# yuki-inaho/APDe-MVS

Measured on AMD Instinct MI355X. Metric: Mpix/s per PatchMatch iteration (ref view, N src) at 1/2/4/8 GPU; depth L1 vs ref, higher is better.
Workload: dtype f32

## Files before the change

### apde-mvs_amd/csrc/apd_kernels.hip

```cpp
#include <hip/hip_runtime.h>

#include <algorithm>
#include <cmath>
#include <cstdio>
#include <cstring>
#include <string>
#include <atomic>
#include <vector>

#include "../../include/apd_hip.h"
#include "apd_device.h"
#include <rocprim/device/device_scan.hpp>

using namespace apd;

#define WAVE 64
#define BLOCK 256
#define APD_PROF_SLOTS 64
#define APD_INSTR 32
#define APD_PROF_SPREAD 64
#define PROF_AT(ev, k) ((ev) + (k) + APD_PROF_SLOTS * (blockIdx.x & (APD_PROF_SPREAD - 1)))
#ifdef APD_PHASE_STAMPS
#define PHASE_STAMP(i)                                                                       \
    do {                                                                                     \
// ... 180 lines not shown
        const unsigned long long m = __ballot(p);
        const int pre = __popcll(m & ((1ull << lane) - 1ull));
        if (lane == 0) wcnt[wv] = __popcll(m);
        __syncthreads();
        int wo = 0;
        for (int k = 0; k < wv; ++k) wo += wcnt[k];
        const int tot = wcnt[0] + wcnt[1] + wcnt[2] + wcnt[3];
        if (mode == 2) {
            if (x < a.W) out[y * a.W + x] = p ? off + wo + pre : -1;
        } else if (p) {
            out[off + wo + pre] = y * a.W + x;
        }
        off += tot;
        __syncthreads();
    }
}

#define TILE_POS 256
#ifndef TILE_SUPER_PX
#define TILE_SUPER_PX 128
#endif
__device__ __forceinline__ void tile_coords(int t, int tiles_x, int tiles_y, int tw, int &tx, int &ty) {
    const int SX = TILE_SUPER_PX ? max(1, TILE_SUPER_PX / tw) : tiles_x;
    const int SY = TILE_SUPER_PX ? max(1, TILE_SUPER_PX / (TILE_POS / tw)) : 1;
    const int sy = t / (SY * tiles_x);
    const int rows = min(SY, tiles_y - SY * sy);
    const int r = t - sy * SY * tiles_x;
    const int sx = r / (rows * SX);
    const int cols = min(SX, tiles_x - SX * sx);
    const int r2 = r - sx * rows * SX;
    tx = SX * sx + r2 % cols;
    ty = SY * sy + r2 / cols;
}
__device__ __forceinline__ void tile_pixel(int tile, int tiles_x, int tiles_y, int tw, int k, int &x, int &y) {
    const int micro = k >> 4, inner = k & 15, mx = tw >> 2;
    const int lx = ((micro % mx) << 2) + (inner & 3);
    const int ly = ((micro / mx) << 2) + (inner >> 2);
    int tx, ty;
    tile_coords(tile, tiles_x, tiles_y, tw, tx, ty);
    x = tx * tw + lx;
    y = ty * (TILE_POS / tw) + ly;
}
__global__ __launch_bounds__(BLOCK) void k_tile_count(Args a, int mode, int colour, int tiles_x, int tw,
                                                    int *__restrict__ counts) {
    int x, y;
    tile_pixel(blockIdx.x, tiles_x, (int)gridDim.x / tiles_x, tw, threadIdx.x, x, y);
    const bool p = x < a.W && y < a.H && list_pred(a, mode, colour, x, y);
    __shared__ int wsum[BLOCK / WAVE];
    const int c = __popcll(__ballot(p));
    if ((threadIdx.x & 63) == 0) wsum[threadIdx.x >> 6] = c;
    __syncthreads();
    if (threadIdx.x == 0) counts[blockIdx.x] = wsum[0] + wsum[1] + wsum[2] + wsum[3];
}
__global__ __launch_bounds__(BLOCK) void k_tile_fill(Args a, int mode, int colour, int tiles_x, int tw,
                                                   const int *__restrict__ offs, int *__restrict__ out) {
    int x, y;
    tile_pixel(blockIdx.x, tiles_x, (int)gridDim.x / tiles_x, tw, threadIdx.x, x, y);
    const bool p = x < a.W && y < a.H && list_pred(a, mode, colour, x, y);
    __shared__ int wcnt[BLOCK / WAVE];
    const int lane = threadIdx.x & 63, wv = threadIdx.x >> 6;
    const unsigned long long m = __ballot(p);
    if (lane == 0) wcnt[wv] = __popcll(m);
    __syncthreads();
    int wo = 0;
    for (int k = 0; k < wv; ++k) wo += wcnt[k];
    const int pos = offs[blockIdx.x] + wo + __popcll(m & ((1ull << lane) - 1ull));
    if (mode == 2) {
        if (x < a.W && y < a.H) out[y * a.W + x] = p ? pos : -1;
    } else if (p) {
        out[pos] = y * a.W + x;
    }
}
__global__ __launch_bounds__(BLOCK) void k_anchor_export(Args a, const int *__restrict__ row_off, short2 *__restrict__ dst) {
    const int y = blockIdx.x;
    __shared__ int wcnt[BLOCK / WAVE];
    int off = row_off[y];
    const int lane = threadIdx.x & 63, wv = threadIdx.x >> 6;
    for (int x0 = 0; x0 < a.W; x0 += BLOCK) {
        const int x = x0 + threadIdx.x;
        const int wi = x < a.W ? a.amap[y * a.W + x] : -1;
        const unsigned long long m = __ballot(wi >= 0);
        if (lane == 0) wcnt[wv] = __popcll(m);
        __syncthreads();
        int wo = 0;
        for (int k = 0; k < wv; ++k) wo += wcnt[k];
        const int tot = wcnt[0] + wcnt[1] + wcnt[2] + wcnt[3];
        if (wi >= 0) {
            const int r = off + wo + __popcll(m & ((1ull << lane) - 1ull));
#pragma unroll
            for (int k = 0; k < 9; ++k) dst[(size_t)r * 9 + k] = a.anchors[(size_t)wi * 9 + k];
// ... 1562 lines not shown
            strong_weight += 1.0f;
        }
    }
    if (dead) return APD_COST_MAX;
    if (strong_weight <= 1e-6f) return center_cost;
    float mx = -1e10f;
#pragma unroll
    for (int t = 0; t < 9; ++t) if (t < ns && sc[t] > mx) mx = sc[t];
    float e[9];
    float sum = 0.0f;
#pragma unroll
    for (int t = 0; t < 9; ++t) {
        if (t < ns) { e[t] = d_expf(sc[t] - mx); sum += e[t]; }
    }
    float acc = 0.0f;
#pragma unroll
    for (int t = 0; t < 9; ++t) {
        if (t < ns) { float w = e[t] / sum; acc = fmaf(w, sc[t], acc); }
    }
    acc = (acc > APD_COST_MAX) ? APD_COST_MAX : acc;
    return (float)(0.25 * (double)center_cost + 0.75 * (double)acc);
}

#ifndef WV_WAVES
#define WV_WAVES 4
#endif
#ifndef WV_CUR_MATCH
#define WV_CUR_MATCH 1
#endif
#ifndef WV_P2_GEOM_BATCH
#define WV_P2_GEOM_BATCH 0
#endif
#define WV_BLOCK (WV_WAVES * WAVE)
template <bool F16, bool SA> struct WvOcc {
#ifdef WV_LDS_OCC
    static constexpr int occ = WV_LDS_OCC;
#else
    static constexpr int occ = F16 ? 4 : 3;
#endif
    static constexpr bool pipe = occ < 4 && WV_CENTRE_PIPE;
};
template <bool F16, bool SA>
__global__ __launch_bounds__(WV_BLOCK, (WvOcc<F16, SA>::occ)) void k_sweep_weak_vm(Args a, const int *__restrict__ list, int count,
                                                                int iter, const float *__restrict__ cand, int wc) {
    const int N = a.N, W = a.W;
    constexpr bool PIPE = WvOcc<F16, SA>::pipe;
    PHASE_BEGIN;
    const bool direct = cand != nullptr;
    WvLdsT<F16, 9, SA> &L = *reinterpret_cast<WvLdsT<F16, 9, SA> *>(apd_dyn_lds);
    wv_init_lut(L);
    float *costL = reinterpret_cast<float *>(&L + 1);
    uint8_t *wts = reinterpret_cast<uint8_t *>(costL + wv_cost_rows(N, direct) * VM_P);
    uint8_t *asl = wts + N * VM_P;
    const int VB = min(WV_P5_CHUNKS, N);
    const int blk = xcd_remap(blockIdx.x, gridDim.x);
    const int first = blk * VM_P;
    const int np = min(VM_P, count - first);
    const int tid = threadIdx.x;
    const int wave = __builtin_amdgcn_readfirstlane(tid >> 6), lane = tid & (WAVE - 1);
    const APD_C Cam &cam0 = a.cams[0];
    const bool geom = a.geom != 0;
    const float gf = a.gf;
    const int p1 = lane;
    const bool pv1 = p1 < np;
    const int c1 = list[first + min(p1, np - 1)];
    const int py1 = c1 / W, px1 = c1 - py1 * W;

    if (pv1) {
        const APD_G short2 *anc = a.anchors + (size_t)a.amap[c1] * 9;
        const int cid = a.sa_any ? a.sa[c1] : 0;
        const bool use_sa = cid != 0;
        if (wave == 0) {
            uint32_t hflag = 0, awin = 0;
            short2 ap[9];
#pragma unroll
            for (int k = 0; k < 9; ++k) ap[k] = anc[k];
            int lab[9], qk[9];
// ... 78 lines not shown
        const float4 pl = L.hyp[h * VM_P + p1];
        const float nv = ncc_new_vm<F16, SA, true, 9, PIPE>(a, L, p1, px1, py1, v + 1, pl, want, nullptr, &nwc, &nwa);
        if (want) val = nv;
        costL[t * VM_P + p1] = val;
    }
    __syncthreads();
    PHASE_STAMP(1);

    const int Gp = WAVE / N;
    const int ppr = WV_WAVES * Gp;
    for (int r0 = 0; r0 < np; r0 += ppr) {
        int g = lane / N;
        const bool lane_ok = g < Gp;
        int v = lane - g * N;
        if (!lane_ok) { g = 0; v = (lane - Gp * N) % N; }
        Group G;
        G.v = v; G.base = g * N; G.slot = g; G.li = 0;
        G.gmask = (N >= 64) ? ~0ull : ((1ull << N) - 1ull);
        const int pr = r0 + wave * Gp + g;
        G.valid = lane_ok && pr < np;
        const int p = min(pr, np - 1);
        const int c = list[first + p];
        const int py = c / W, px = c - py * W;
        const uint32_t hflag = L.flags[p] & 0x1FFu;
        float prior = 0.0f;
        const uint32_t asv = asl[v * VM_P + p];
#pragma unroll
        for (int i = 0; i < 8; ++i) {
            const int pk = L.anc[(i + 1) * VM_P + p];
            if (pk >= 0) prior += ((asv >> i) & 1u) ? 0.9f : 0.1f;
        }
        float ca[8];
        if (direct) {
            const size_t wi = (size_t)a.amap[c];
#pragma unroll
            for (int h = 0; h < 8; ++h)
                ca[h] = ((hflag >> h) & 1u) ? cand[((size_t)v * 8 + h) * (size_t)wc + wi] : ((h == 0 && v == 0) ? 2.0f : 0.0f);
        } else {
#pragma unroll
            for (int h = 0; h < 8; ++h) ca[h] = costL[(h * N + v) * VM_P + p];
        }
        Rng rg(a.seed_lo, a.seed_hi, (uint32_t)c, ord_weak(iter));
        const int w = view_selection(ca, prior, iter, rg, G, N);
        const uint32_t tsel = group_bits(w > 0, G);
        float gval[8];
#ifdef APD_PHASE_STAMPS
        const long long tg0_ = clock64();
#endif
#if WV_P2_GEOM_BATCH
        if (geom && w > 0) {
            GeomHead gh[8];
            float sdep[8];
#pragma unroll
            for (int j = 0; j < 8; ++j) {
                float P[3];
                geom_point(a, px, py, L.hyp[j * VM_P + p], P);
                gh[j] = geom_head(a, v + 1, P);
            }
#pragma unroll
            for (int j = 0; j < 8; ++j) sdep[j] = ((hflag >> j) & 1u) ? a.depth[gh[j].idx] : 0.0f;
#pragma unroll
            for (int j = 0; j < 8; ++j)
                gval[j] = ((hflag >> j) & 1u) ? fmaf(gf, geom_tail(a, px, py, v + 1, gh[j], sdep[j]), ca[j]) : fmaf(gf, 3.0f, ca[j]);
        } else {
#pragma unroll
            for (int j = 0; j < 8; ++j) gval[j] = ca[j];
        }
#else
        const bool share_p = geom && N >= 8;
        float Pv[3] = {0.0f, 0.0f, 0.0f};
// ... 801 lines not shown
    float4 *dst = reinterpret_cast<float4 *>(pcost + (size_t)i0 * Np);
    for (int j = threadIdx.x; j < nq; j += BLOCK) dst[j] = src[j];
}

__device__ __forceinline__ float gp_combine(float cc, const float (&sc)[8]) {
    if (cc < 0.0f) return APD_COST_MAX;
    const float center_cost = cc;
    uint32_t pm = 0;
    float strong_weight = 0.0f;
#pragma unroll
    for (int k = 0; k < 8; ++k)
        if (sc[k] >= 0.0f) { pm |= 1u << k; strong_weight += 1.0f; }
    if (strong_weight <= 1e-6f) return center_cost;
    float mx = -1e10f;
#pragma unroll
    for (int k = 0; k < 8; ++k) if (((pm >> k) & 1u) && sc[k] > mx) mx = sc[k];
    float e[8];
    float sum = 0.0f;
#pragma unroll
    for (int k = 0; k < 8; ++k) {
        e[k] = 0.0f;
        if ((pm >> k) & 1u) { e[k] = d_expf(sc[k] - mx); sum += e[k]; }
    }
    float acc = 0.0f;
#pragma unroll
    for (int k = 0; k < 8; ++k)
        if ((pm >> k) & 1u) { const float w = e[k] / sum; acc = fmaf(w, sc[k], acc); }
    acc = (acc > APD_COST_MAX) ? APD_COST_MAX : acc;
    return (float)(0.25 * (double)center_cost + 0.75 * (double)acc);
}

template <bool F16, bool SA>
__global__ __launch_bounds__(PK_BLOCK, PK_MINW) void k_weak_cand_g(Args a, const int *__restrict__ list, int count,
                                                          const uint8_t *__restrict__ cbw, float *__restrict__ out, int wc) {
    using TT = FastTex<F16, true>;
    using RT = typename std::conditional<F16, _Float16, float>::type;
    __shared__ RT cref[36 * VM_P];
    __shared__ float csr[VM_P], csrr[VM_P];
    __shared__ uint64_t cmask[VM_P];
    __shared__ uint8_t cws[VM_P], cbits[VM_P];
    __shared__ int anc0[VM_P];
    const int N = a.N, W = a.W, H = a.H;
    const int blk = xcd_remap(blockIdx.x, gridDim.x);
    const int first = blk * VM_P;
    const int np = min(VM_P, count - first);
    const int tid = threadIdx.x;
    const int wave = __builtin_amdgcn_readfirstlane(tid >> 6), lane = tid & (WAVE - 1);
    const int p1 = lane;
    const bool pv1 = p1 < np;
    const int c1 = list[first + min(p1, np - 1)];
    const int py1 = c1 / W, px1 = c1 - py1 * W;
    const int wi1 = a.amap[c1];
    const int cid = a.sa_any ? (int)a.sa[c1] : 0;
    const APD_G short2 *anc1 = a.anchors + (size_t)wi1 * 9;
    if (wave == 0) {
        int a0 = -1;
        uint32_t cb = 0;
        if (pv1) {
            const short2 z = anc1[0];
            const bool ok = !(z.x == -1 || z.y == -1) && (cid == 0 || (int)a.sa[z.x + z.y * W] == cid);
            a0 = ok ? ((int)(uint16_t)z.x | ((int)z.y << 16)) : -1;
            cb = cbw[wi1];
        }
        anc0[p1] = a0;
        cbits[p1] = (uint8_t)cb;
    }
    __syncthreads();
// ... 37 lines not shown
        const short2 ap = anc1[h + 1];
        pl = a.plane[ap.x + ap.y * W];
    }
    const int pk0 = anc0[p1];
    const uint64_t tm = SA ? cmask[p1] : ~0ull;
    uint32_t nlive = 0;
    for (int v = 0; v < N; ++v) {
        const int s = v + 1;
        const TT T(a, s);
        const SrcTex<F16> Q(a, s);
        const Hom Hm = homography(a, s, pl);
        float ptx, pty;
        project(Hm, (float)px1, (float)py1, ptx, pty);
        const bool alive = want && !(ptx >= (float)W || ptx < 0.0f || pty >= (float)H || pty < 0.0f);
        const bool has = alive && pk0 >= 0;
        const int ax = has ? (pk0 & 0xFFFF) : px1, ay = has ? (pk0 >> 16) : py1;
        bool live = has, dead = !alive;
        if (has) {
            float asx, asy;
            project(Hm, (float)ax, (float)ay, asx, asy);
            if (asx < 0 || asy < 0 || asx >= (float)W || asy >= (float)H) { live = false; dead = true; }
        }
        float center_cost = 0.0f;
        if (__ballot(live)) {
            const bool fast = live && window_rcp_ok(Hm, (float)(ax - 5), (float)(ay - 5));
            float ss = 0.0f, sss = 0.0f, srs = 0.0f;
            ncc_new_window<F16, 6, 2, PK_PIPE>(a, &cref[p1], VM_P, tm, Hm, ax, ay, live, fast, T, Q, ss, sss, srs);
            if (live) {
                const float wsum = (float)cws[p1];
                if (wsum != 0.0f) center_cost = ncc_finalize(csr[p1], csrr[p1], ss, sss, srs, wsum);
            }
        }
        nlive += live;
        if (want) out[((size_t)v * 8 + h) * (size_t)wc + wi1] = dead ? -1.0f : center_cost;
    }
    if (a.evals) wave_count(a.evals, 6, nlive);
}
#define COMB_STRIDE 33
__global__ __launch_bounds__(BLOCK) void k_weak_cand_comb(Args a, const int *__restrict__ list, int count,
                                                          const uint8_t *__restrict__ cbw, const uint8_t *__restrict__ wmw,
                                                          const uint32_t *__restrict__ pidx,
                                                          const float *__restrict__ pcost, float *__restrict__ out, int wc) {
    __shared__ uint32_t sid[VM_P * COMB_STRIDE];
    const int b = xcd_remap(blockIdx.x, gridDim.x);
    const int h0 = (b & 1) << 2, hl = threadIdx.x >> 6, h = h0 + hl;
    const int g0 = (b >> 1) * VM_P;
    const int lane = threadIdx.x & (WAVE - 1);
    for (int e = threadIdx.x; e < VM_P * 8; e += BLOCK) {
        const int slot = e >> 3, k = e & 7;
        if (g0 + slot < count) {
            const int wi2 = a.amap[list[g0 + slot]];
            const uint4 q = *reinterpret_cast<const uint4 *>(pidx + (size_t)wi2 * 64 + k * 8 + h0);
            uint32_t *d = &sid[slot * COMB_STRIDE + k * 4];
            d[0] = q.x; d[1] = q.y; d[2] = q.z; d[3] = q.w;
        }
    }
    __syncthreads();
    const int i = g0 + lane;
    if (i >= count) return;
    const int wi = a.amap[list[i]];
    if (!((cbw[wi] >> h) & 1u)) return;
    const int N = a.N, Np = (N + 3) & ~3;
    const uint32_t wm = wmw[wi];
    const float4 *pc4[8];
#pragma unroll
    for (int k = 0; k < 8; ++k) {
        const uint32_t id = ((wm >> k) & 1u) ? sid[lane * COMB_STRIDE + k * 4 + hl] : 0u;
        pc4[k] = reinterpret_cast<const float4 *>(pcost + (size_t)id * Np);
    }
    for (int v0 = 0; v0 < N; v0 += 4) {
        float4 q[8];
#pragma unroll
        for (int k = 0; k < 8; ++k) q[k] = ((wm >> k) & 1u) ? pc4[k][v0 >> 2] : make_float4(-1.0f, -1.0f, -1.0f, -1.0f);
#pragma unroll
        for (int dv = 0; dv < 4; ++dv) {
            const int v = v0 + dv;
            if (v >= N) break;
            float sc[8];
#pragma unroll
            for (int k = 0; k < 8; ++k) sc[k] = dv == 0 ? q[k].x : dv == 1 ? q[k].y : dv == 2 ? q[k].z : q[k].w;
            float *o = out + ((size_t)v * 8 + h) * (size_t)wc + wi;
            *o = gp_combine(*o, sc);
        }
    }
}

__global__ __launch_bounds__(BLOCK) void k_depth_normal(Args a) {
    const int c = blockIdx.x * BLOCK + threadIdx.x;
    if (c >= a.HW) return;
    const int py = c / a.W, px = c - py * a.W;
    float4 p = a.plane[c];
    p.w = depth_from_plane(a.cams[0], p, px, py);
    a.plane[c] = to_world(a.cams[0], p);
}

__global__ __launch_bounds__(BLOCK) void k_filter(Args a, const int *__restrict__ list, int count) {
    const int li = blockIdx.x * BLOCK + threadIdx.x;
    if (li >= count) return;
    const int W = a.W, H = a.H;
    const int c = list[li];
    const int py = c / W, px = c - py * W;
    if (a.cost[c] < 0.001f) return;
    float f[21];
    int n = 0;
    f[n++] = a.plane[c].w;
    const int left = c - 1, leftleft = c - 3, up = c - W, upup = c - 3 * W;
    const int down = c + W, downdown = c + 3 * W, right = c + 1, rightright = c + 3;
    const uint8_t *wk = a.weak;
#define FADD(cond, idx) if ((cond) && wk[(idx)] == APD_STRONG) f[n++] = a.plane[(idx)].w
    FADD(py > 0, up);
    FADD(py > 2, upup);
    FADD(py > 4, upup - W * 2);
    FADD(py < H - 1, down);
    FADD(py < H - 3, downdown);
// ... 686 lines not shown
    size_t bytes = 0;
};

const char *g_global_err = "";
std::string g_global_err_store;

void set_global_err(const std::string &s) {
    g_global_err_store = s;
    g_global_err = g_global_err_store.c_str();
}

}

struct apd_ctx {
    int device = 0;
    hipStream_t stream = nullptr;
    hipStream_t side[2] = {nullptr, nullptr};
    hipEvent_t ev_fork = nullptr, ev_side[2] = {nullptr, nullptr};
    bool overlap = true;
    std::string err;
    DevBuf imgs, quad, depth, views, cams, plane, cost, sel, sel2, vw, weak, conf, sa, amap, anchors, reliable, nearest,
        fit, curve, lists, rowcnt, rowoff, totals, near_off, dargs, evals, near_ring, near_g, wcand, lrs, wcur, arec, ga_stage,
        wlist, gp_cb, gp_cnt, gp_cur, gp_refs, gp_ccnt, gp_cbase, gp_plist, gp_pidx, gp_pcost, gp_tmp, dpairs, gp_cls;
    int n_near = 0;
    int host_stat[4] = {0, 0, 0, 0};
    int near_levels = 0;
    Args args{};
    bool loaded = false, prepared = false;
    int optional_fallbacks = 0;
    bool prep_timed = false;
    int dw_tile_w = 8;
    int tile_w = 16;
    bool cand_pairs = true;
    bool gp_on = false;
    bool ga_split = true;
    bool rec_on = false;
    bool dtex = true;
    int gp_np = 0;
    bool gp_one_pass = true;
    bool gp_async = true;
    bool gp_pending = false;
    size_t gp_pcap = 0;
    int ncu = 256;
    bool gp_place = true;
    bool gp_small = true;
    int gp_cap_factor = 2;
    bool lr_handover = true;
    bool wcur_on = true;
    bool wcur_fresh = false;
    int weak_count = 0;
    size_t lrs_need = 0;
    int cnt[4] = {0, 0, 0, 0};
    size_t list_cap = 0;
    bool want_curve = false;
    apd_params params{};
    hipEvent_t ev[16] = {};
    apd_timing timing{};
    struct ProfEv {
        hipEvent_t e0, e1;
        int kind;
        int64_t px;
    };
    bool prof = false;
    std::vector<ProfEv> prof_ev;
    std::vector<hipEvent_t> prof_pool;
};
// ... 165 lines not shown
    if (hipStreamCreateWithFlags(&ctx->stream, hipStreamNonBlocking) != hipSuccess) {
        set_global_err("hipStreamCreate failed");
        delete ctx;
        return nullptr;
    }
    for (auto &e : ctx->ev) (void)hipEventCreateWithFlags(&e, hipEventDisableSystemFence);
    int prio_least = 0, prio_greatest = 0;
    (void)hipDeviceGetStreamPriorityRange(&prio_least, &prio_greatest);
    const bool low_side = !(getenv("APD_SIDE_PRIORITY") && atoi(getenv("APD_SIDE_PRIORITY")) == 0);
    if (low_side && prio_least <= 0 && prio_greatest < 0) {
        hipStream_t hi = nullptr;
        if (hipStreamCreateWithPriority(&hi, hipStreamNonBlocking, prio_greatest) == hipSuccess) {
            (void)hipStreamDestroy(ctx->stream);
            ctx->stream = hi;
        }
    }
    if (getenv("APD_DEBUG_PRIO")) fprintf(stderr, "apd: stream priorities least %d greatest %d\n", prio_least, prio_greatest);
    for (auto &ss : ctx->side) {
        int prio = 0;
        if (low_side && prio_least > 0 && &ss == &ctx->side[0]) prio = prio_least;
        if (low_side && prio_least <= 0 && prio_greatest < 0 && &ss == &ctx->side[1]) prio = prio_greatest;
        if (hipStreamCreateWithPriority(&ss, hipStreamNonBlocking, prio) != hipSuccess) {
            set_global_err("hipStreamCreate failed");
            for (auto &t : ctx->side) if (t) (void)hipStreamDestroy(t);
            (void)hipStreamDestroy(ctx->stream);
            delete ctx;
            return nullptr;
        }
    }
    (void)hipEventCreateWithFlags(&ctx->ev_fork, hipEventDisableTiming);
    for (auto &e : ctx->ev_side) (void)hipEventCreateWithFlags(&e, hipEventDisableTiming);
    ctx->overlap = getenv("APD_NO_OVERLAP") == nullptr;
    ctx->cand_pairs = getenv("APD_NO_CAND_PAIRS") == nullptr;
    ctx->ga_split = getenv("APD_NO_GA_SPLIT") == nullptr;
    ctx->lr_handover = getenv("APD_NO_LR_HANDOVER") == nullptr;
    ctx->wcur_on = getenv("APD_NO_WCUR") == nullptr;
    ctx->dtex = getenv("APD_NO_DTEX") == nullptr;
    ctx->gp_one_pass = getenv("APD_GP_TWO_PASS") == nullptr;
    ctx->gp_small = getenv("APD_GP_NO_SMALL") == nullptr;
    ctx->gp_place = getenv("APD_GP_FILL") == nullptr;
    ctx->gp_async = getenv("APD_GP_SYNC") == nullptr && ctx->gp_one_pass && ctx->gp_small && ctx->gp_place;
    {
        int n = 0;
        if (hipDeviceGetAttribute(&n, hipDeviceAttributeMultiprocessorCount, device) == hipSuccess && n > 0) ctx->ncu = n;
    }
    if (const char *e = getenv("APD_GP_CAP_FACTOR")) ctx->gp_cap_factor = std::max(0, std::min(8, atoi(e)));

    if (const char *e = getenv("APD_DW_TILE_W")) {
        const int t = atoi(e);
        if (t == 1 || t == 2 || t == 4 || t == 8 || t == 16 || t == 32 || t == 64) ctx->dw_tile_w = t;
    }
    if (const char *e = getenv("APD_TILE_W")) {
        const int t = atoi(e);
        if (t == 4 || t == 8 || t == 16 || t == 32 || t == 64) ctx->tile_w = t;
    }
    const void *vm_kernels[] = {
        (const void *)k_sweep_strong_vm<true, false>, (const void *)k_sweep_strong_vm<false, false>,
        (const void *)k_sweep_strong_vm<true, true>, (const void *)k_sweep_strong_vm<false, true>,
        (const void *)k_sweep_weak_vm<true, false>, (const void *)k_sweep_weak_vm<false, false>,
        (const void *)k_sweep_weak_vm<true, true>, (const void *)k_sweep_weak_vm<false, true>,
        (const void *)k_depth_to_weak_vm<true, false>, (const void *)k_depth_to_weak_vm<false, false>,
        (const void *)k_depth_to_weak_vm<true, true>, (const void *)k_depth_to_weak_vm<false, true>,
        (const void *)k_depth_to_weak_vm<true, false, true>, (const void *)k_depth_to_weak_vm<true, true, true>,
        (const void *)k_local_refine_vm<true, false>, (const void *)k_local_refine_vm<false, false>,
        (const void *)k_local_refine_vm<true, true>, (const void *)k_local_refine_vm<false, true>,
        (const void *)k_random_init_vm<true, false, false>, (const void *)k_random_init_vm<false, false, false>,
// ... 234 lines not shown
    if (ctx->lr_handover) {
        const int tw = ctx->dw_tile_w, th = VM_P / tw;
        const size_t slots = (size_t)(((W + tw - 1) / tw) * ((H + th - 1) / th)) * VM_P;
        const size_t need = (size_t)11 * N * slots * sizeof(float) * (P.geom_consistency ? 2 : 1);
        if (ctx->lrs.p && ctx->lrs.bytes != need) {
            (void)hipFree(ctx->lrs.p);
            ctx->lrs.p = nullptr;
            ctx->lrs.bytes = 0;
        }
        size_t free_b = 0, total_b = 0;
        const size_t spare = (size_t)4 << 30;
        if (!ctx->lrs.p && hipMemGetInfo(&free_b, &total_b) == hipSuccess && free_b > spare && need <= free_b - spare) {
            if (ensure(ctx, ctx->lrs, need) != APD_OK) {
                (void)hipGetLastError();
                ctx->err.clear();
            }
        }
        if (ctx->lrs.p) ctx->lrs_need = need;
    }
    ctx->params = P;
    ctx->loaded = true;
    return APD_OK;
}

static void tile_count_scan(apd_ctx *ctx, int mode, int colour, int *total_dev) {
    Args &a = ctx->args;
    const int tw = ctx->tile_w, th = TILE_POS / tw;
    const int tx = (a.W + tw - 1) / tw, ty = (a.H + th - 1) / th;
    hipLaunchKernelGGL(k_tile_count, dim3(tx * ty), dim3(BLOCK), 0, ctx->stream, a, mode, colour, tx, tw,
                       (int *)ctx->rowcnt.p);
    hipLaunchKernelGGL(k_list_scan, dim3(1), dim3(1024), 0, ctx->stream, (const int *)ctx->rowcnt.p, tx * ty,
                       (int *)ctx->rowoff.p, total_dev);
}
static int build_tile_list(apd_ctx *ctx, int mode, int colour, int *out, int *total_dev) {
    Args &a = ctx->args;
    const int tw = ctx->tile_w, th = TILE_POS / tw;
    const int tx = (a.W + tw - 1) / tw, ty = (a.H + th - 1) / th;
    tile_count_scan(ctx, mode, colour, total_dev);
    hipLaunchKernelGGL(k_tile_fill, dim3(tx * ty), dim3(BLOCK), 0, ctx->stream, a, mode, colour, tx, tw,
                       (const int *)ctx->rowoff.p, out);
    return check_launch(ctx, "tile list build");
}
static int build_list(apd_ctx *ctx, int mode, int colour, int *out, int *total_dev) {
    Args &a = ctx->args;
    hipStream_t s = ctx->stream;
    hipLaunchKernelGGL(k_list_count, dim3(a.H), dim3(BLOCK), 0, s, a, mode, colour, (int *)ctx->rowcnt.p);
    hipLaunchKernelGGL(k_list_scan, dim3(1), dim3(1024), 0, s, (const int *)ctx->rowcnt.p, a.H, (int *)ctx->rowoff.p,
                       total_dev);
    hipLaunchKernelGGL(k_list_fill, dim3(a.H), dim3(BLOCK), 0, s, a, mode, colour, (const int *)ctx->rowoff.p, out);
    return check_launch(ctx, "list build");
}

static int *list_ptr(apd_ctx *ctx, int which) {
    int *base = (int *)ctx->lists.p;
    size_t off = 0;
    for (int i = 0; i < which; ++i) off += (size_t)ctx->cnt[i];
    return base + off;
}


static bool test_enomem_hook(apd_ctx *ctx) {
    static std::atomic<int> n{0};
    const char *e = getenv("APD_TEST_LIB_ENOMEM_AT");
    if (!e || ++n != atoi(e)) return false;
    ctx->err = "hipMalloc failed (APD_TEST_LIB_ENOMEM_AT)";
    return true;
}

static int exclusive_scan_int(apd_ctx *ctx, const int *in, int *out, size_t n) {
    size_t tb = 0;
    HIP_OK(ctx, rocprim::exclusive_scan(nullptr, tb, in, out, 0, n, rocprim::plus<int>(), ctx->stream));
    if (!try_ensure(ctx, ctx->gp_tmp, tb)) return APD_ENOMEM;
    HIP_OK(ctx, rocprim::exclusive_scan(ctx->gp_tmp.p, tb, in, out, 0, n, rocprim::plus<int>(), ctx->stream));
    return APD_OK;
}

static int build_global_pairs(apd_ctx *ctx, int nw) {
    Args &a = ctx->args;
    hipStream_t s = ctx->stream;
    const size_t HW = (size_t)a.HW, wc = (size_t)std::max(ctx->weak_count, 1);
    ctx->gp_on = false;
    ctx->gp_np = 0;
    if (!try_ensure(ctx, ctx->gp_cnt, (HW + 1) * sizeof(int)) || !try_ensure(ctx, ctx->gp_cur, (HW + 1) * sizeof(int)) ||
        !try_ensure(ctx, ctx->gp_refs, (size_t)nw * 8 * sizeof(uint32_t)) ||
        !try_ensure(ctx, ctx->gp_pidx, wc * 64 * sizeof(uint32_t)) || !try_ensure(ctx, ctx->gp_cb, 2 * wc))
        return APD_OK;
    int *cnt = (int *)ctx->gp_cnt.p, *cur = (int *)ctx->gp_cur.p;
    HIP_OK(ctx, hipMemsetAsync(cnt, 0, (HW + 1) * sizeof(int), s));
    uint32_t *loc = (uint32_t *)ctx->gp_pidx.p;
    if (ctx->gp_place)
// ... 127 lines not shown
    const size_t U = HW > (size_t)ctx->weak_count ? HW - (size_t)ctx->weak_count : 1;
    const size_t cap2 = U + 1 + (size_t)nw * 8 / GP_SPLIT + 1;
    const int *ctr = (const int *)ctx->gp_cls.p + 2 * (U + 1) + 2 * cap2;
    int h[8] = {};
    HIP_OK(ctx, hipMemcpyAsync(h, ctr, 8 * sizeof(int), hipMemcpyDeviceToHost, ctx->stream));
    HIP_OK(ctx, hipStreamSynchronize(ctx->stream));
    const int npairs = h[5];
    if (h[4] != 0 || npairs < 0 || (size_t)npairs > ctx->gp_pcap) {
        if (npairs < 0 || (size_t)npairs > ctx->gp_pcap) ctx->gp_cap_factor = 8;
        const bool rec = ctx->rec_on;
        int st = build_global_pairs(ctx, nw);
        if (st) return st;
        if (!rec) ctx->gp_on = false;
        return check_launch(ctx, "pair table");
    }
    if (npairs > 0 && !try_ensure(ctx, ctx->gp_pcost, (size_t)npairs * ((ctx->args.N + 3) & ~3) * sizeof(float))) {
        ctx->gp_on = false;
        return APD_OK;
    }
    ctx->gp_np = npairs;
    return APD_OK;
}

int32_t apd_stage_prepare(apd_ctx *ctx) {
    if (!ctx || !ctx->loaded) return APD_ESTATE;
    (void)hipSetDevice(ctx->device);
    Args &a = ctx->args;
    hipStream_t s = ctx->stream;
    const unsigned gpx = blocks_for((size_t)a.HW, BLOCK);
    int st;
    ctx->gp_on = false;
    (void)hipEventRecord(ctx->ev[0], s);
    if (a.use_apd) {
        if ((st = build_tile_list(ctx, 2, 0, (int *)ctx->amap.p, (int *)ctx->totals.p + 4))) return st;
        if (ctx->near_levels) {
            hipLaunchKernelGGL(k_near_columns, dim3(blocks_for((size_t)ctx->near_levels * a.W, BLOCK)), dim3(BLOCK), 0, s, a,
                               ctx->near_levels, (uint8_t *)ctx->near_g.p);
            hipLaunchKernelGGL(k_find_nearest_rows, dim3(gpx), dim3(BLOCK), 0, s, a, (const uint8_t *)ctx->near_g.p,
                               (const int *)ctx->near_ring.p);
        } else {
            hipLaunchKernelGGL(k_find_nearest, dim3(gpx), dim3(BLOCK), 0, s, a, ctx->n_near);
        }
        {
            Args ag = a;
            ag.evals = (ctx->prof && ctx->evals.p) ? (APD_G unsigned long long *)ctx->evals.p : nullptr;
            const size_t wc = (size_t)std::max(ctx->weak_count, 1);
            uint32_t *stage = (ctx->ga_split && ctx->weak_count > 0 &&
                               try_ensure(ctx, ctx->ga_stage, (size_t)GA_STAGE_W * wc * sizeof(uint32_t)))
                                  ? (uint32_t *)ctx->ga_stage.p : nullptr;
            if (stage) {
                hipLaunchKernelGGL(k_gen_anchors<true>, dim3(gpx), dim3(BLOCK), 0, s, ag, stage, (int)wc);
                hipLaunchKernelGGL(k_gen_anchors_fit, dim3(blocks_for(wc, GA_FIT_WAVES)), dim3(GA_FIT_WAVES * WAVE), 0, s, a,
                                   (const uint32_t *)stage, (int)wc);
            } else {
                hipLaunchKernelGGL(k_gen_anchors<false>, dim3(gpx), dim3(BLOCK), 0, s, ag, stage, (int)wc);
            }
        }
        hipLaunchKernelGGL(k_neighbour_update, dim3(gpx), dim3(BLOCK), 0, s, a);
        if ((st = check_launch(ctx, "anchors"))) return st;
    }
    (void)hipEventRecord(ctx->ev[1], s);
    hipStream_t sri = s;
    if (ctx->overlap) {
        HIP_OK(ctx, hipEventRecord(ctx->ev_fork, s));
        HIP_OK(ctx, hipStreamWaitEvent(ctx->side[0], ctx->ev_fork, 0));
        sri = ctx->side[0];
    }
    {
        const int tw = ctx->dw_tile_w, th = VM_P / tw;
        const unsigned nb = (unsigned)(((a.W + tw - 1) / tw) * ((a.H + th - 1) / th));
        if (a.use_apd) {
            if (a.sa_any) {
                if (a.tex_f16) hipLaunchKernelGGL((k_random_init_vm<true, true, true>), dim3(nb), dim3(VM_BLOCK), (ri_lds_bytes<true, true>(a.N) + sa_lds_bytes(a)), sri, a, tw);
                else hipLaunchKernelGGL((k_random_init_vm<false, true, true>), dim3(nb), dim3(VM_BLOCK), (ri_lds_bytes<false, true>(a.N) + sa_lds_bytes(a)), sri, a, tw);
            } else {
                if (a.tex_f16) hipLaunchKernelGGL((k_random_init_vm<true, true, false>), dim3(nb), dim3(VM_BLOCK), (ri_lds_bytes<true, true>(a.N)), sri, a, tw);
                else hipLaunchKernelGGL((k_random_init_vm<false, true, false>), dim3(nb), dim3(VM_BLOCK), (ri_lds_bytes<false, true>(a.N)), sri, a, tw);
            }
        } else {
            if (a.sa_any) {
                if (a.tex_f16) hipLaunchKernelGGL((k_random_init_vm<true, false, true>), dim3(nb), dim3(VM_BLOCK), (ri_lds_bytes<true, false>(a.N) + sa_lds_bytes(a)), sri, a, tw);
                else hipLaunchKernelGGL((k_random_init_vm<false, false, true>), dim3(nb), dim3(VM_BLOCK), (ri_lds_bytes<false, false>(a.N) + sa_lds_bytes(a)), sri, a, tw);
            } else {
                if (a.tex_f16) hipLaunchKernelGGL((k_random_init_vm<true, false, false>), dim3(nb), dim3(VM_BLOCK), (ri_lds_bytes<true, false>(a.N)), sri, a, tw);
                else hipLaunchKernelGGL((k_random_init_vm<false, false, false>), dim3(nb), dim3(VM_BLOCK), (ri_lds_bytes<false, false>(a.N)), sri, a, tw);
            }
        }
        if ((st = check_launch(ctx, "k_random_init"))) return st;
        (void)hipEventRecord(ctx->ev[15], sri);
        if (ctx->overlap) HIP_OK(ctx, hipEventRecord(ctx->ev_side[0], sri));
    }
    {
        int *tot = (int *)ctx->totals.p;
        const int modes[4][2] = {{0, 0}, {0, 1}, {1, 0}, {1, 1}};
        for (int i = 0; i < 4; ++i) tile_count_scan(ctx, modes[i][0], modes[i][1], tot + i);
        int host_tot[4];
        HIP_OK(ctx, hipMemcpyAsync(host_tot, tot, 4 * sizeof(int), hipMemcpyDeviceToHost, s));
        HIP_OK(ctx, hipStreamSynchronize(s));
        for (int i = 0; i < 4; ++i) ctx->cnt[i] = host_tot[i];
        for (int i = 0; i < 4; ++i) {
            if ((st = build_tile_list(ctx, modes[i][0], modes[i][1], list_ptr(ctx, i), tot + i))) return st;
        }
        if (a.use_apd && ctx->cand_pairs && ctx->cnt[2] + ctx->cnt[3] > 0) {
            const size_t wc = (size_t)std::max(ctx->weak_count, 1);
            if (test_enomem_hook(ctx)) return APD_ENOMEM;
            if ((st = ensure(ctx, ctx->wcand, (size_t)a.N * 8 * wc * sizeof(float)))) return st;
            if ((st = ensure(ctx, ctx->wlist, (size_t)(ctx->cnt[2] + ctx->cnt[3]) * sizeof(int)))) return st;
            if ((st = build_tile_list(ctx, 1, 2, (int *)ctx->wlist.p, tot + 5))) return st;
            (void)hipEventRecord(ctx->ev[14], s);
            if ((size_t)a.HW < (1u << 25) && a.W < 32768 && a.H < 32768 &&
                (st = ctx->gp_async ? build_global_pairs_async(ctx, ctx->cnt[2] + ctx->cnt[3])
                                    : build_global_pairs(ctx, ctx->cnt[2] + ctx->cnt[3])))
                return st;
        } else {
            (void)hipEventRecord(ctx->ev[14], s);
        }
        ctx->rec_on = false;
        a.arec = nullptr;
        if (a.use_apd && ctx->gp_on && (ctx->gp_np > 0 || ctx->gp_pending)) {
            const size_t rb = (size_t)a.HW * (a.sa_any ? 2 : 1) * (a.tex_f16 ? 2 : 4) * sizeof(uint4);
            if (try_ensure(ctx, ctx->arec, rb)) {
                a.arec = devptr<decltype(a.arec)>(ctx->arec.p);
                const unsigned g = blocks_for((size_t)a.HW, BLOCK);
                if (a.tex_f16) hipLaunchKernelGGL(k_anchor_rec<true>, dim3(g), dim3(BLOCK), 0, s, a, (uint4 *)ctx->arec.p);
                else hipLaunchKernelGGL(k_anchor_rec<false>, dim3(g), dim3(BLOCK), 0, s, a, (uint4 *)ctx->arec.p);
                if ((st = check_launch(ctx, "k_anchor_rec"))) return st;
                ctx->rec_on = true;
            } else {
                ctx->gp_on = false;
            }
        }
    }
    (void)hipEventRecord(ctx->ev[2], s);
    if (ctx->overlap) HIP_OK(ctx, hipStreamWaitEvent(s, ctx->ev_side[0], 0));
    HIP_OK(ctx, hipMemcpyAsync(ctx->sel.p, ctx->sel2.p, (size_t)a.HW * sizeof(uint32_t), hipMemcpyDeviceToDevice, s));
    (void)hipEventRecord(ctx->ev[3], s);
    if ((st = finish_global_pairs(ctx, ctx->cnt[2] + ctx->cnt[3]))) return st;
    ctx->prep_timed = true;
    ctx->wcur_fresh = a.wcur != nullptr;
    ctx->prepared = true;
    return APD_OK;
// ... 30 lines not shown
    Args &a = ctx->args;
    hipStream_t s = ctx->stream;
    int st;
    APD_G unsigned long long *evals = (ctx->prof && ctx->evals.p) ? (APD_G unsigned long long *)ctx->evals.p : nullptr;
    for (int colour = 0; colour < 2; ++colour) {
        const int n = ctx->cnt[colour];
        if (n <= 0) continue;
        hipEvent_t e0 = prof_begin(ctx);
        Args ak = a;
        ak.evals = evals;
        if (!(ctx->wcur_fresh && iter == 0)) ak.wcur = nullptr;
        LAUNCH_TEX_SA(k_sweep_strong_vm, dim3(blocks_for((size_t)n, VM_P)), dim3(VM_BLOCK), vm_lds_bytes(a.N, ctx->args.tex_f16 != 0) + sa_lds_bytes(a), s,
                      ak, (const int *)list_ptr(ctx, colour), n, iter);
        prof_end(ctx, e0, APD_PROF_STRONG_SWEEP, n);
        if ((st = check_launch(ctx, "k_sweep_strong"))) return st;
    }
    if (a.use_apd) {
        hipEvent_t ewp = prof_begin(ctx);
        hipStream_t sr = s, sg = s;
        if (ctx->overlap) {
            HIP_OK(ctx, hipEventRecord(ctx->ev_fork, s));
            HIP_OK(ctx, hipStreamWaitEvent(ctx->side[0], ctx->ev_fork, 0));
            HIP_OK(ctx, hipStreamWaitEvent(ctx->side[1], ctx->ev_fork, 0));
            sr = ctx->side[0];
            sg = ctx->side[1];
        }
        hipEvent_t e0 = prof_begin(ctx, sr);
        hipLaunchKernelGGL(k_ransac_fit, dim3(blocks_for((size_t)a.HW, BLOCK)), dim3(BLOCK), 0, sr, a, iter);
        prof_end(ctx, e0, APD_PROF_RANSAC_FIT, a.HW, sr);
        if (ctx->overlap) HIP_OK(ctx, hipEventRecord(ctx->ev_side[0], sr));
        const int nw = ctx->cnt[2] + ctx->cnt[3];
        const int wc = std::max(ctx->weak_count, 1);
        const float *cand = nullptr;
        if (ctx->cand_pairs && nw > 0 && ctx->gp_on) {
            if (ctx->wcand.bytes < (size_t)a.N * 8 * (size_t)wc * sizeof(float) || ctx->wlist.bytes < (size_t)nw * sizeof(int)) {
                ctx->err = "candidate cost buffers not sized by apd_stage_prepare";
                return APD_ESTATE;
            }
            Args ac = a;
            ac.evals = evals;
            {
                hipEvent_t e1 = prof_begin(ctx, sg);
                if (ctx->gp_np > 0)
                    LAUNCH_TEX_SA(k_gp_cost, dim3(blocks_for((size_t)ctx->gp_np, BLOCK)), dim3(BLOCK), gp_cost_lds_bytes(a.N), sg, ac,
                               (const int2 *)ctx->gp_plist.p, ctx->gp_np, (float *)ctx->gp_pcost.p);
                prof_end(ctx, e1, APD_PROF_GP_COST, ctx->gp_np, sg);
                if (ctx->overlap) HIP_OK(ctx, hipEventRecord(ctx->ev_side[1], sg));
                e1 = prof_begin(ctx);
                LAUNCH_TEX_SA(k_weak_cand_g, dim3(blocks_for((size_t)nw, VM_P)), dim3(PK_BLOCK), 0, s, ac, (const int *)ctx->wlist.p, nw,
                              (const uint8_t *)ctx->gp_cb.p, (float *)ctx->wcand.p, wc);
                prof_end(ctx, e1, APD_PROF_WEAK_CAND_G, nw);
                if (ctx->overlap) HIP_OK(ctx, hipStreamWaitEvent(s, ctx->ev_side[1], 0));
                e1 = prof_begin(ctx);
                hipLaunchKernelGGL(k_weak_cand_comb, dim3(2 * blocks_for((size_t)nw, VM_P)), dim3(BLOCK), 0, s, ac,
                                   (const int *)ctx->wlist.p, nw, (const uint8_t *)ctx->gp_cb.p, (const uint8_t *)ctx->gp_cb.p + wc,
                                   (const uint32_t *)ctx->gp_pidx.p, (const float *)ctx->gp_pcost.p, (float *)ctx->wcand.p, wc);
                prof_end(ctx, e1, APD_PROF_WEAK_CAND_COMB, nw);
            }
            cand = (const float *)ctx->wcand.p;
        }
        if (ctx->overlap) HIP_OK(ctx, hipStreamWaitEvent(s, ctx->ev_side[0], 0));
        for (int colour = 0; colour < 2; ++colour) {
            const int n = ctx->cnt[2 + colour];
            if (n <= 0) continue;
            Args aw = a;
            aw.evals = evals;
            if (!(ctx->wcur_fresh && iter == 0)) aw.wcur = nullptr;
            e0 = prof_begin(ctx);
            const bool direct = cand != nullptr;
            LAUNCH_TEX_SA(k_sweep_weak_vm, dim3(blocks_for((size_t)n, VM_P)), dim3(WV_BLOCK),
                          (ctx->args.tex_f16 ? (ctx->args.sa_any ? wv_lds_bytes<true, 9, true>(a.N, direct) : wv_lds_bytes<true, 9, false>(a.N, direct))
                                             : (ctx->args.sa_any ? wv_lds_bytes<false, 9, true>(a.N, direct) : wv_lds_bytes<false, 9, false>(a.N, direct))),
                          s,
                          aw, (const int *)list_ptr(ctx, 2 + colour), n, iter, cand, wc);
            prof_end(ctx, e0, APD_PROF_WEAK_SWEEP, n);
        }
        prof_end(ctx, ewp, APD_PROF_WEAK_PATH, ctx->cnt[2] + ctx->cnt[3]);
        if ((st = check_launch(ctx, "weak sweep"))) return st;
    }
    ctx->wcur_fresh = false;
    return APD_OK;
}

int32_t apd_stage_finish(apd_ctx *ctx) {
    if (!ctx || !ctx->prepared) return APD_ESTATE;
    (void)hipSetDevice(ctx->device);
    Args a = ctx->args;
    hipStream_t s = ctx->stream;
    int st;
    const unsigned gpx = blocks_for((size_t)a.HW, BLOCK);
    hipLaunchKernelGGL(k_depth_normal, dim3(gpx), dim3(BLOCK), 0, s, a);
    for (int colour = 0; colour < 2; ++colour) {
        const int n = ctx->cnt[colour];
        if (n > 0)
            hipLaunchKernelGGL(k_filter, dim3(blocks_for((size_t)n, BLOCK)), dim3(BLOCK), 0, s, a,
                               (const int *)list_ptr(ctx, colour), n);
    }
    if (ctx->want_curve && ctx->curve.p) a.curve = devptr<decltype(a.curve)>(ctx->curve.p);
    a.lr_ncc = nullptr;
    a.lr_geo = nullptr;
    if (ctx->lr_handover && ctx->lrs_need > 0 && ctx->lrs.p && ctx->lrs.bytes >= ctx->lrs_need) {
        const size_t plane = ctx->lrs_need / (sizeof(float) * (a.geom ? 2 : 1));
        a.lr_ncc = devptr<decltype(a.lr_ncc)>(ctx->lrs.p);
        a.lr_geo = a.geom ? devptr<decltype(a.lr_geo)>((float *)ctx->lrs.p + plane) : nullptr;
    }
    {
        const int tw = ctx->dw_tile_w, th = VM_P / tw;
// ... 311 lines not shown
```

Baseline: 64.94.

## Merge weak sweeps into one launch and store candidate costs group-major

By default the weak-pixel sweep becomes a single launch over the combined weak list instead of one launch per checkerboard colour, and the per-colour weak lists are no longer built. Candidate costs are stored in a block-grouped (group-major) layout indexed by list position, so each block's reads and writes of candidate costs are contiguous. An optional quad-ordered tile pixel mapping is added behind an environment flag. The goal is less launch overhead, fewer list builds, and better memory coalescing. The trade-off is dropping the red/black colour separation in the weak update, which changes update order and may affect convergence or depth results.

```diff
diff --git a/apde-mvs_amd/csrc/apd_kernels.hip b/apde-mvs_amd/csrc/apd_kernels.hip
--- a/apde-mvs_amd/csrc/apd_kernels.hip
+++ b/apde-mvs_amd/csrc/apd_kernels.hip
@@ -236,10 +236,17 @@
     tx = SX * sx + r2 % cols;
     ty = SY * sy + r2 / cols;
 }
-__device__ __forceinline__ void tile_pixel(int tile, int tiles_x, int tiles_y, int tw, int k, int &x, int &y) {
+__host__ __device__ __forceinline__ bool tile_quad_ok(int tw) { return tw >= 8 && TILE_POS / tw >= 8; }
+__device__ __forceinline__ void tile_pixel(int tile, int tiles_x, int tiles_y, int tw, int k, int &x, int &y, bool quad = false) {
     const int micro = k >> 4, inner = k & 15, mx = tw >> 2;
-    const int lx = ((micro % mx) << 2) + (inner & 3);
-    const int ly = ((micro / mx) << 2) + (inner >> 2);
+    int mcol = micro % mx, mrow = micro / mx;
+    if (quad) {
+        const int q = micro >> 2, i = micro & 3, qx = mx >> 1;
+        mcol = ((q % qx) << 1) + (i & 1);
+        mrow = ((q / qx) << 1) + (i >> 1);
+    }
+    const int lx = (mcol << 2) + (inner & 3);
+    const int ly = (mrow << 2) + (inner >> 2);
     int tx, ty;
     tile_coords(tile, tiles_x, tiles_y, tw, tx, ty);
     x = tx * tw + lx;
@@ -257,9 +264,9 @@
     if (threadIdx.x == 0) counts[blockIdx.x] = wsum[0] + wsum[1] + wsum[2] + wsum[3];
 }
 __global__ __launch_bounds__(BLOCK) void k_tile_fill(Args a, int mode, int colour, int tiles_x, int tw,
-                                                   const int *__restrict__ offs, int *__restrict__ out) {
+                                                   const int *__restrict__ offs, int *__restrict__ out, int quad) {
     int x, y;
-    tile_pixel(blockIdx.x, tiles_x, (int)gridDim.x / tiles_x, tw, threadIdx.x, x, y);
+    tile_pixel(blockIdx.x, tiles_x, (int)gridDim.x / tiles_x, tw, threadIdx.x, x, y, quad != 0);
     const bool p = x < a.W && y < a.H && list_pred(a, mode, colour, x, y);
     __shared__ int wcnt[BLOCK / WAVE];
     const int lane = threadIdx.x & 63, wv = threadIdx.x >> 6;
@@ -1888,6 +1895,10 @@
 #define WV_P2_GEOM_BATCH 0
 #endif
 #define WV_BLOCK (WV_WAVES * WAVE)
+__device__ __forceinline__ size_t cand_at(bool gm, int N, int v, int h, int wc, int wi, int li) {
+    return gm ? ((size_t)(li / VM_P) * (size_t)(N * 8) + (size_t)(v * 8 + h)) * VM_P + (size_t)(li % VM_P)
+              : ((size_t)v * 8 + h) * (size_t)wc + (size_t)wi;
+}
 template <bool F16, bool SA> struct WvOcc {
 #ifdef WV_LDS_OCC
     static constexpr int occ = WV_LDS_OCC;
@@ -1898,7 +1909,7 @@
 };
 template <bool F16, bool SA>
 __global__ __launch_bounds__(WV_BLOCK, (WvOcc<F16, SA>::occ)) void k_sweep_weak_vm(Args a, const int *__restrict__ list, int count,
-                                                                int iter, const float *__restrict__ cand, int wc) {
+                                                                int iter, const float *__restrict__ cand, int wc, int gm) {
     const int N = a.N, W = a.W;
     constexpr bool PIPE = WvOcc<F16, SA>::pipe;
     PHASE_BEGIN;
@@ -2043,10 +2054,11 @@
         }
         float ca[8];
         if (direct) {
-            const size_t wi = (size_t)a.amap[c];
+            const float *cp = cand + cand_at(gm != 0, N, v, 0, wc, gm ? 0 : a.amap[c], first + p);
+            const size_t hs = gm ? (size_t)VM_P : (size_t)wc;
 #pragma unroll
             for (int h = 0; h < 8; ++h)
-                ca[h] = ((hflag >> h) & 1u) ? cand[((size_t)v * 8 + h) * (size_t)wc + wi] : ((h == 0 && v == 0) ? 2.0f : 0.0f);
+                ca[h] = ((hflag >> h) & 1u) ? cp[h * hs] : ((h == 0 && v == 0) ? 2.0f : 0.0f);
         } else {
 #pragma unroll
             for (int h = 0; h < 8; ++h) ca[h] = costL[(h * N + v) * VM_P + p];
@@ -2914,7 +2926,7 @@
 
 template <bool F16, bool SA>
 __global__ __launch_bounds__(PK_BLOCK, PK_MINW) void k_weak_cand_g(Args a, const int *__restrict__ list, int count,
-                                                          const uint8_t *__restrict__ cbw, float *__restrict__ out, int wc) {
+                                                          const uint8_t *__restrict__ cbw, float *__restrict__ out, int wc, int gm) {
     using TT = FastTex<F16, true>;
     using RT = typename std::conditional<F16, _Float16, float>::type;
     __shared__ RT cref[36 * VM_P];
@@ -3018,7 +3030,7 @@
             }
         }
         nlive += live;
-        if (want) out[((size_t)v * 8 + h) * (size_t)wc + wi1] = dead ? -1.0f : center_cost;
+        if (want) out[cand_at(gm != 0, N, v, h, wc, wi1, first + p1)] = dead ? -1.0f : center_cost;
     }
     if (a.evals) wave_count(a.evals, 6, nlive);
 }
@@ -3026,7 +3038,7 @@
 __global__ __launch_bounds__(BLOCK) void k_weak_cand_comb(Args a, const int *__restrict__ list, int count,
                                                           const uint8_t *__restrict__ cbw, const uint8_t *__restrict__ wmw,
                                                           const uint32_t *__restrict__ pidx,
-                                                          const float *__restrict__ pcost, float *__restrict__ out, int wc) {
+                                                          const float *__restrict__ pcost, float *__restrict__ out, int wc, int gm) {
     __shared__ uint32_t sid[VM_P * COMB_STRIDE];
     const int b = xcd_remap(blockIdx.x, gridDim.x);
     const int h0 = (b & 1) << 2, hl = threadIdx.x >> 6, h = h0 + hl;
@@ -3065,7 +3077,7 @@
             float sc[8];
 #pragma unroll
             for (int k = 0; k < 8; ++k) sc[k] = dv == 0 ? q[k].x : dv == 1 ? q[k].y : dv == 2 ? q[k].z : q[k].w;
-            float *o = out + ((size_t)v * 8 + h) * (size_t)wc + wi;
+            float *o = out + cand_at(gm != 0, N, v, h, wc, wi, i);
             *o = gp_combine(*o, sc);
         }
     }
@@ -3818,6 +3830,9 @@
     int dw_tile_w = 8;
     int tile_w = 16;
     bool cand_pairs = true;
+    bool weak_per_colour = false;
+    bool weak_quad = false;
+    bool cand_gm = true;
     bool gp_on = false;
     bool ga_split = true;
     bool rec_on = false;
@@ -4049,6 +4064,9 @@
     for (auto &e : ctx->ev_side) (void)hipEventCreateWithFlags(&e, hipEventDisableTiming);
     ctx->overlap = getenv("APD_NO_OVERLAP") == nullptr;
     ctx->cand_pairs = getenv("APD_NO_CAND_PAIRS") == nullptr;
+    ctx->weak_per_colour = getenv("APD_WEAK_PER_COLOUR") != nullptr;
+    ctx->weak_quad = getenv("APD_WEAK_QUAD") != nullptr;
+    ctx->cand_gm = getenv("APD_NO_CAND_GROUP_MAJOR") == nullptr && !ctx->weak_per_colour;
     ctx->ga_split = getenv("APD_NO_GA_SPLIT") == nullptr;
     ctx->lr_handover = getenv("APD_NO_LR_HANDOVER") == nullptr;
     ctx->wcur_on = getenv("APD_NO_WCUR") == nullptr;
@@ -4349,13 +4367,13 @@
     hipLaunchKernelGGL(k_list_scan, dim3(1), dim3(1024), 0, ctx->stream, (const int *)ctx->rowcnt.p, tx * ty,
                        (int *)ctx->rowoff.p, total_dev);
 }
-static int build_tile_list(apd_ctx *ctx, int mode, int colour, int *out, int *total_dev) {
+static int build_tile_list(apd_ctx *ctx, int mode, int colour, int *out, int *total_dev, bool quad = false) {
     Args &a = ctx->args;
     const int tw = ctx->tile_w, th = TILE_POS / tw;
     const int tx = (a.W + tw - 1) / tw, ty = (a.H + th - 1) / th;
     tile_count_scan(ctx, mode, colour, total_dev);
     hipLaunchKernelGGL(k_tile_fill, dim3(tx * ty), dim3(BLOCK), 0, ctx->stream, a, mode, colour, tx, tw,
-                       (const int *)ctx->rowoff.p, out);
+                       (const int *)ctx->rowoff.p, out, (quad && tile_quad_ok(tw)) ? 1 : 0);
     return check_launch(ctx, "tile list build");
 }
 static int build_list(apd_ctx *ctx, int mode, int colour, int *out, int *total_dev) {
@@ -4373,6 +4391,9 @@
     size_t off = 0;
     for (int i = 0; i < which; ++i) off += (size_t)ctx->cnt[i];
     return base + off;
+}
+static size_t wcand_bytes(int N, size_t wc, int nw) {
+    return (size_t)N * 8 * std::max(wc, (size_t)blocks_for((size_t)nw, VM_P) * VM_P) * sizeof(float);
 }
 
 
@@ -4566,7 +4587,7 @@
     ctx->gp_on = false;
     (void)hipEventRecord(ctx->ev[0], s);
     if (a.use_apd) {
-        if ((st = build_tile_list(ctx, 2, 0, (int *)ctx->amap.p, (int *)ctx->totals.p + 4))) return st;
+        if ((st = build_tile_list(ctx, 2, 0, (int *)ctx->amap.p, (int *)ctx->totals.p + 4, ctx->weak_quad))) return st;
         if (ctx->near_levels) {
             hipLaunchKernelGGL(k_near_columns, dim3(blocks_for((size_t)ctx->near_levels * a.W, BLOCK)), dim3(BLOCK), 0, s, a,
                                ctx->near_levels, (uint8_t *)ctx->near_g.p);
@@ -4632,15 +4653,18 @@
         HIP_OK(ctx, hipMemcpyAsync(host_tot, tot, 4 * sizeof(int), hipMemcpyDeviceToHost, s));
         HIP_OK(ctx, hipStreamSynchronize(s));
         for (int i = 0; i < 4; ++i) ctx->cnt[i] = host_tot[i];
-        for (int i = 0; i < 4; ++i) {
+        for (int i = 0; i < (ctx->weak_per_colour ? 4 : 2); ++i) {
             if ((st = build_tile_list(ctx, modes[i][0], modes[i][1], list_ptr(ctx, i), tot + i))) return st;
         }
-        if (a.use_apd && ctx->cand_pairs && ctx->cnt[2] + ctx->cnt[3] > 0) {
+        const int nw = ctx->cnt[2] + ctx->cnt[3];
+        if (a.use_apd && nw > 0) {
+            if ((st = ensure(ctx, ctx->wlist, (size_t)nw * sizeof(int)))) return st;
+            if ((st = build_tile_list(ctx, 1, 2, (int *)ctx->wlist.p, tot + 5, ctx->weak_quad))) return st;
+        }
+        if (a.use_apd && ctx->cand_pairs && nw > 0) {
             const size_t wc = (size_t)std::max(ctx->weak_count, 1);
             if (test_enomem_hook(ctx)) return APD_ENOMEM;
-            if ((st = ensure(ctx, ctx->wcand, (size_t)a.N * 8 * wc * sizeof(float)))) return st;
-            if ((st = ensure(ctx, ctx->wlist, (size_t)(ctx->cnt[2] + ctx->cnt[3]) * sizeof(int)))) return st;
-            if ((st = build_tile_list(ctx, 1, 2, (int *)ctx->wlist.p, tot + 5))) return st;
+            if ((st = ensure(ctx, ctx->wcand, wcand_bytes(a.N, wc, nw)))) return st;
             (void)hipEventRecord(ctx->ev[14], s);
             if ((size_t)a.HW < (1u << 25) && a.W < 32768 && a.H < 32768 &&
                 (st = ctx->gp_async ? build_global_pairs_async(ctx, ctx->cnt[2] + ctx->cnt[3])
@@ -4737,8 +4761,9 @@
         const int nw = ctx->cnt[2] + ctx->cnt[3];
         const int wc = std::max(ctx->weak_count, 1);
         const float *cand = nullptr;
+        const int gm = ctx->cand_gm ? 1 : 0;
         if (ctx->cand_pairs && nw > 0 && ctx->gp_on) {
-            if (ctx->wcand.bytes < (size_t)a.N * 8 * (size_t)wc * sizeof(float) || ctx->wlist.bytes < (size_t)nw * sizeof(int)) {
+            if (ctx->wcand.bytes < wcand_bytes(a.N, (size_t)wc, nw) || ctx->wlist.bytes < (size_t)nw * sizeof(int)) {
                 ctx->err = "candidate cost buffers not sized by apd_stage_prepare";
                 return APD_ESTATE;
             }
@@ -4753,20 +4778,25 @@
                 if (ctx->overlap) HIP_OK(ctx, hipEventRecord(ctx->ev_side[1], sg));
                 e1 = prof_begin(ctx);
                 LAUNCH_TEX_SA(k_weak_cand_g, dim3(blocks_for((size_t)nw, VM_P)), dim3(PK_BLOCK), 0, s, ac, (const int *)ctx->wlist.p, nw,
-                              (const uint8_t *)ctx->gp_cb.p, (float *)ctx->wcand.p, wc);
+                              (const uint8_t *)ctx->gp_cb.p, (float *)ctx->wcand.p, wc, gm);
                 prof_end(ctx, e1, APD_PROF_WEAK_CAND_G, nw);
                 if (ctx->overlap) HIP_OK(ctx, hipStreamWaitEvent(s, ctx->ev_side[1], 0));
                 e1 = prof_begin(ctx);
                 hipLaunchKernelGGL(k_weak_cand_comb, dim3(2 * blocks_for((size_t)nw, VM_P)), dim3(BLOCK), 0, s, ac,
                                    (const int *)ctx->wlist.p, nw, (const uint8_t *)ctx->gp_cb.p, (const uint8_t *)ctx->gp_cb.p + wc,
-                                   (const uint32_t *)ctx->gp_pidx.p, (const float *)ctx->gp_pcost.p, (float *)ctx->wcand.p, wc);
+                                   (const uint32_t *)ctx->gp_pidx.p, (const float *)ctx->gp_pcost.p, (float *)ctx->wcand.p, wc, gm);
                 prof_end(ctx, e1, APD_PROF_WEAK_CAND_COMB, nw);
             }
             cand = (const float *)ctx->wcand.p;
         }
         if (ctx->overlap) HIP_OK(ctx, hipStreamWaitEvent(s, ctx->ev_side[0], 0));
-        for (int colour = 0; colour < 2; ++colour) {
-            const int n = ctx->cnt[2 + colour];
+        if (!ctx->weak_per_colour && nw > 0 && ctx->wlist.bytes < (size_t)nw * sizeof(int)) {
+            ctx->err = "WEAK lists not built by apd_stage_prepare";
+            return APD_ESTATE;
+        }
+        for (int colour = 0; colour < (ctx->weak_per_colour ? 2 : 1); ++colour) {
+            const int n = ctx->weak_per_colour ? ctx->cnt[2 + colour] : nw;
+            const int *wl = ctx->weak_per_colour ? (const int *)list_ptr(ctx, 2 + colour) : (const int *)ctx->wlist.p;
             if (n <= 0) continue;
             Args aw = a;
             aw.evals = evals;
@@ -4777,7 +4807,7 @@
                           (ctx->args.tex_f16 ? (ctx->args.sa_any ? wv_lds_bytes<true, 9, true>(a.N, direct) : wv_lds_bytes<true, 9, false>(a.N, direct))
                                              : (ctx->args.sa_any ? wv_lds_bytes<false, 9, true>(a.N, direct) : wv_lds_bytes<false, 9, false>(a.N, direct))),
                           s,
-                          aw, (const int *)list_ptr(ctx, 2 + colour), n, iter, cand, wc);
+                          aw, wl, n, iter, cand, wc, gm);
             prof_end(ctx, e0, APD_PROF_WEAK_SWEEP, n);
         }
         prof_end(ctx, ewp, APD_PROF_WEAK_PATH, ctx->cnt[2] + ctx->cnt[3]);
```

Result: faster. 67.88, median of 6 (+4.5%).
